# lr40/marl-scheduling

Measured on AMD Instinct MI355X. Metric: agent-env-steps/sec (whole node), 8 agents×8 cores×16384 envs, 1/2/4/8 MI355X, higher is better.
Workload: dtype int8/f32

## Files before the change

marl-scheduling_amd/csrc/env_kernels.hip:

```cpp
#include <hip/hip_runtime.h>
#include <stdlib.h>
#include <string.h>

#include "ms_layout.h"
#include "ms_act.h"

#pragma clang fp contract(off)

namespace ms {

__device__ __forceinline__ void wave_sync() {
    __builtin_amdgcn_fence(__ATOMIC_RELEASE, "wavefront");
    __builtin_amdgcn_wave_barrier();
    __builtin_amdgcn_fence(__ATOMIC_ACQUIRE, "wavefront");
}

#ifdef MS_PHASE_TIMING
constexpr int kProbeSlots = 65536;
__device__ unsigned long long g_phase_cycles[kProbeSlots][16];
__device__ unsigned long long g_wave_span[kProbeSlots][2];
__device__ unsigned long long g_free_cycles[kProbeSlots][5];
#define MS_MARK(k)                                                     \
    do {                                                               \
        const uint64_t t_now = __builtin_amdgcn_s_memtime();          \
        t_acc[k] += t_now - t_prev;                                    \
        t_prev = t_now;                                                \
    } while (0)
#else
#define MS_MARK(k) \
    do {           \
    } while (0)
#endif

template <int LPE>
struct Lanes {
    int gl;
    int gbase;
    __device__ explicit Lanes(int lane) : gl(lane & (LPE - 1)), gbase(lane & ~(LPE - 1)) {}
    __device__ __forceinline__ uint64_t ballot(bool p) const {
        const uint64_t m = __ballot(p);
        return LPE == 64 ? m : (m >> gbase) & ((1ull << (LPE & 63)) - 1ull);
    }
    __device__ __forceinline__ uint32_t shfl(uint32_t v, int src) const { return (uint32_t)__shfl((int)v, gbase + src); }
};


__device__ __forceinline__ uint32_t mt_temper(uint32_t y) {
    y ^= (y >> 11);
    y ^= (y << 7) & 0x9d2c5680u;
    y ^= (y << 15) & 0xefc60000u;
    y ^= (y >> 18);
    return y;
}

__device__ __forceinline__ uint32_t mt_step(uint32_t hi_src, uint32_t lo_src, uint32_t xsrc) {
    const uint32_t y = (hi_src & 0x80000000u) | (lo_src & 0x7fffffffu);
    return xsrc ^ (y >> 1) ^ ((y & 1u) ? 0x9908b0dfu : 0u);
}

__device__ __forceinline__ void mt_phase_range(int ph, int& lo, int& hi) {
    lo = ph * (kMtN - kMtM);
    hi = ph < 2 ? (ph + 1) * (kMtN - kMtM) : kMtN - 1;
}

__device__ void mt_twist_lds_wave(uint32_t* st, int lane) {
    for (int ph = 0; ph < 3; ph++) {
        int lo, hi;
        mt_phase_range(ph, lo, hi);
        for (int c0 = lo; c0 < hi; c0 += kWave) {
            const int i = c0 + lane;
            uint32_t v = 0;
            if (i < hi) v = mt_step(st[i], st[i + 1], st[ph == 0 ? i + kMtM : i + (kMtM - kMtN)]);
            wave_sync();
            if (i < hi) st[i] = v;
            wave_sync();
        }
    }
    if (lane == 0) st[kMtN - 1] = mt_step(st[kMtN - 1], st[0], st[kMtM - 1]);
    wave_sync();
}

__device__ void mt_twist_into_successor(uint32_t* mt_env, uint32_t sel, uint8_t* lds, int lane) {
    uint32_t* st = reinterpret_cast<uint32_t*>(lds);
    const uint32_t h = sel & 1u;
    const uint32_t* cur = mt_env + h * kMtN;
    uint32_t* nxt = mt_env + (h ^ 1u) * kMtN;
    for (int i = lane; i < kMtN; i += kWave) st[i] = cur[i];
    wave_sync();
    mt_twist_lds_wave(st, lane);
    for (int i = lane; i < kMtN; i += kWave) nxt[i] = st[i];
    __builtin_amdgcn_fence(__ATOMIC_RELEASE, "workgroup");
    __builtin_amdgcn_fence(__ATOMIC_ACQUIRE, "workgroup");
    wave_sync();
}

template <int LPE>
__device__ void mt_refill_groups(uint32_t* mt, int64_t e0, uint64_t need, uint32_t sel, uint8_t* lds, int lane) {
    while (need) {
        const int src = __ffsll((unsigned long long)need) - 1;
        need &= need - 1;
        mt_twist_into_successor(mt + (e0 + src / LPE) * 2 * kMtN, (uint32_t)__shfl((int)sel, src), lds, lane);
    }
}

template <int LPE>
__device__ void mt_refill_next(uint32_t* mt, const uint8_t* recs, const Geom& P, int64_t slot, bool active,
                               uint8_t* lds, int lane) {
    const int gl = lane & (LPE - 1);
    const int64_t e0 = slot * (kWave / LPE);
    uint32_t sel = 0;
    if (active && gl == 0) sel = *reinterpret_cast<const uint32_t*>(recs + (e0 + lane / LPE) * P.rec_bytes + 12);
    mt_refill_groups<LPE>(mt, e0, __ballot(active && gl == 0 && !(sel & 2u)), sel, lds, lane);
}

__device__ __forceinline__ void mt_commit(int fin, int32_t* mti, uint32_t* sel) {
    const uint32_t h = *sel & 1u;
    if (fin > 2 * kMtN) {
        *sel = h;
        *mti = fin - 2 * kMtN;
    } else if (fin > kMtN) {
        *sel = h ^ 1u;
        *mti = fin - kMtN;
    } else {
        *sel = h | 2u;
        *mti = fin;
    }
}

__device__ __forceinline__ uint32_t mt_ld(const uint32_t* p) {
    return __hip_atomic_load(const_cast<uint32_t*>(p), __ATOMIC_RELAXED, __HIP_MEMORY_SCOPE_AGENT);
}
__device__ __forceinline__ void mt_st(uint32_t* p, uint32_t v) {
    __hip_atomic_store(p, v, __ATOMIC_RELAXED, __HIP_MEMORY_SCOPE_AGENT);
}

template <int LPE>
__device__ void mt_twist_from(uint32_t* cur, const uint32_t* nxt, int gl) {
    for (int i = gl; i < kMtN; i += LPE) mt_st(cur + i, nxt[i]);
    __builtin_amdgcn_fence(__ATOMIC_ACQ_REL, "workgroup");
    for (int ph = 0; ph < 3; ph++) {
        int lo, hi;
        mt_phase_range(ph, lo, hi);
        for (int c0 = lo; c0 < hi; c0 += LPE) {
            const int i = c0 + gl;
            uint32_t v = 0;
            if (i < hi) v = mt_step(mt_ld(cur + i), mt_ld(cur + i + 1), mt_ld(cur + (ph == 0 ? i + kMtM : i + (kMtM - kMtN))));
            __builtin_amdgcn_fence(__ATOMIC_ACQ_REL, "workgroup");
            if (i < hi) mt_st(cur + i, v);
            __builtin_amdgcn_fence(__ATOMIC_ACQ_REL, "workgroup");
        }
    }
    if (gl == 0) mt_st(cur + kMtN - 1, mt_step(mt_ld(cur + kMtN - 1), mt_ld(cur), mt_ld(cur + kMtM - 1)));
    __builtin_amdgcn_fence(__ATOMIC_ACQ_REL, "workgroup");
}

template <int LPE>
struct MtStream {
    uint32_t* cur;
    uint32_t* nxt;
    int mti0;
    int wb, wend;
    int p;
    bool fell_back;
    bool overrun;
    bool store;
    uint32_t v;

    __device__ void init(uint32_t* mt_env, uint32_t sel, int mti, bool active) {
        cur = mt_env + (sel & 1u) * kMtN;
        nxt = mt_env + ((sel & 1u) ^ 1u) * kMtN;
        mti0 = mti;
        wb = wend = p = 0;
        fell_back = false;
        overrun = false;
        store = active;
// ... 1368 lines not shown
        const int owner = (int)reinterpret_cast<const int8_t*>(sl + g.s_rec + g.o_core_owner)[c];
        const bool v = ge < EPW && e < E && owner > 0;
        const uint32_t* crow = reinterpret_cast<const uint32_t*>(sl + g.s_scratch) + c * nw;
        const int c0 = 2 * g4, c1 = 2 * g4 + 1;
        const u4v x = bytes_to_bf16(crow[c0 < nw ? c0 : nw - 1], crow[c1 < nw ? c1 : nw - 1]);
        acc_a[0] = (f4){0, 0, 0, 0};
        acc_a[0] = mfma_bf16(wa.hi[0], x, acc_a[0]);
        acc_a[0] = mfma_bf16(wa.mid[0], x, acc_a[0]);
        acc_a[0] = mfma_bf16(wa.lo[0], x, acc_a[0]);
        acc_a[1] = acc_a[0];
        const int64_t item = e * Ua + (owner - 1) * C + c;
        u_a[0] = philox_u(item, fa.acc.row_base, fa.acc_offset);
        u_a[1] = 0.f;
        row_a[0] = v ? (int)item : -1;
        row_a[1] = -1;
    }
    ho.run2(acc_o, Ao, g4, u_o, act_o, lp_o);
    ha.run2(acc_a, Aa, g4, u_a, act_a, lp_a);
    store(fa.off_action, fa.off_logprob, row_o, act_o, lp_o);
    store(fa.acc_action, fa.acc_logprob, row_a, act_a, lp_a);
    for (int t0 = 32; t0 < EPW * Uo; t0 += 32) {
        offer_rows(t0, acc_o, row_o, u_o);
        ho.run2(acc_o, Ao, g4, u_o, act_o, lp_o);
        store(fa.off_action, fa.off_logprob, row_o, act_o, lp_o);
    }
    const float S = __uint_as_float(s_tab[0]);
    const int last_nz = (int)s_tab[1];
    {
        const int ge = lane / Ua, u = lane - ge * Ua, a = u / C, c = u - a * C;
        const int64_t e = e0 + ge;
        const uint8_t* sl = smem_all + (size_t)(ge < EPW ? ge : 0) * g.s_total;
        const bool in = lane < EPW * Ua && e < E;
        const int owner = (int)reinterpret_cast<const int8_t*>(sl + g.s_rec + g.o_core_owner)[c];
        if (in && owner != a + 1) {
            const int64_t item = e * Ua + u;
            const float target = philox_u(item, fa.acc.row_base, fa.acc_offset) * S;
            int cnt = 0;
#pragma unroll
            for (int step = 16; step >= 1; step >>= 1)
                if (cnt + step <= 16 && s_cum[cnt + step - 1] <= target) cnt += step;
            const int act = cnt >= Aa ? last_nz : cnt;
            fa.acc_action[item] = (int8_t)act;
            fa.acc_logprob[item] = s_lp[act];
        }
    }
}

template <int LPE, bool EXT, bool CMP, class SH>
__global__ void __launch_bounds__(64, 4) k_env_step(Params P, int64_t E, uint8_t* recs, uint32_t* mt, Liab* liab,
                                                 StepIO io) {
#ifdef MS_PHASE_TIMING
    const uint64_t rt_start = __builtin_amdgcn_s_memrealtime();
#endif
    if (io.span && threadIdx.x == 0) {
        io.span[4 * blockIdx.x] = __builtin_amdgcn_s_memrealtime();
        io.span[4 * blockIdx.x + 2] = __builtin_amdgcn_s_memtime();
    }
    env_round<LPE, EXT, CMP, SH>(P, E, recs, mt, liab, io, blockIdx.x);
    if (io.span && threadIdx.x == 0) {
        io.span[4 * blockIdx.x + 3] = __builtin_amdgcn_s_memtime();
        io.span[4 * blockIdx.x + 1] = __builtin_amdgcn_s_memrealtime();
    }
#ifdef MS_PHASE_TIMING
    if (threadIdx.x == 0) {
        g_wave_span[blockIdx.x % kProbeSlots][0] = rt_start;
        g_wave_span[blockIdx.x % kProbeSlots][1] = __builtin_amdgcn_s_memrealtime();
    }
#endif
}

template <int LPE, class SH, bool MET = false>
__global__ void __launch_bounds__(64, 4) k_env_step_act(Params P, int64_t E, uint8_t* recs, uint32_t* mt, Liab* liab,
                                                     StepIO io, FusedAct fa) {
    if (io.span && threadIdx.x == 0) {
        io.span[4 * blockIdx.x] = __builtin_amdgcn_s_memrealtime();
        io.span[4 * blockIdx.x + 2] = __builtin_amdgcn_s_memtime();
    }
    env_round<LPE, false, true, SH, MET>(P, E, recs, mt, liab, io, blockIdx.x);
    fused_act<LPE, SH>(P, E, fa, blockIdx.x);
    if (io.span && threadIdx.x == 0) {
        io.span[4 * blockIdx.x + 3] = __builtin_amdgcn_s_memtime();
        io.span[4 * blockIdx.x + 1] = __builtin_amdgcn_s_memrealtime();
    }
}

template <class T>
__device__ __forceinline__ T* advance(T* p, int64_t bytes) {
    return p ? reinterpret_cast<T*>(reinterpret_cast<uintptr_t>(p) + bytes) : p;
}
struct RolloutArgs {
    Params P;
    int64_t E;
    uint8_t* recs;
    uint32_t* mt;
    Liab* liab;
    StepIO io;
    FusedAct fa;
    RoundStride st;
    int n_rounds, act_last;
};
template <int LPE, class SH, bool MET = false>
__global__ void __launch_bounds__(64, 2) k_env_rollout_act(RolloutArgs A0) {
    unsigned long long* span = A0.io.span;
    if (span && threadIdx.x == 0) {
        span[4 * blockIdx.x] = __builtin_amdgcn_s_memrealtime();
        span[4 * blockIdx.x + 2] = __builtin_amdgcn_s_memtime();
    }
    const int n_rounds = A0.n_rounds;
    for (int t = 0; t < n_rounds; t++) {
        auto ka = __builtin_amdgcn_kernarg_segment_ptr();
        asm volatile("" : "+s"(ka));
        const RolloutArgs& A = *(const RolloutArgs*)ka;
        int lane = threadIdx.x;
        asm volatile("" : "+v"(lane));
        const RoundStride& st = A.st;
        StepIO io = A.io;
        io.span = nullptr;
        io.act_acc = advance(io.act_acc, t * st.act_acc);
        io.act_off = advance(io.act_off, t * st.act_off);
        io.obs_crow = advance(io.obs_crow, t * st.obs_crow);
        io.obs_cown = advance(io.obs_cown, t * st.obs_cown);
        io.obs_off = advance(io.obs_off, t * st.obs_off);
        io.rew_offer = advance(io.rew_offer, t * st.rew_offer);
        io.rew_acc = advance(io.rew_acc, t * st.rew_acc);
        io.rew_agent = advance(io.rew_agent, t * st.rew_agent);
        io.rew_auct = advance(io.rew_auct, t * st.rew_auct);
        env_round<LPE, false, true, SH, MET, MET>(A.P, A.E, A.recs, A.mt, A.liab, io, blockIdx.x, lane);
        if (t + 1 < n_rounds || A.act_last) {
            FusedAct fa = A.fa;
            fa.off_action = advance(fa.off_action, t * st.off_action);
            fa.off_logprob = advance(fa.off_logprob, t * st.off_logprob);
            fa.acc_action = advance(fa.acc_action, t * st.acc_action);
            fa.acc_logprob = advance(fa.acc_logprob, t * st.acc_logprob);
            fa.off_offset += (uint64_t)t * st.offset_step;
            fa.acc_offset += (uint64_t)t * st.offset_step;
            fused_act<LPE, SH>(A.P, A.E, fa, blockIdx.x, lane);
        }
        __builtin_amdgcn_fence(__ATOMIC_RELEASE, "workgroup");
        __builtin_amdgcn_fence(__ATOMIC_ACQUIRE, "workgroup");
        wave_sync();
    }
    if (span && threadIdx.x == 0) {
        span[4 * blockIdx.x + 3] = __builtin_amdgcn_s_memtime();
        span[4 * blockIdx.x + 1] = __builtin_amdgcn_s_memrealtime();
    }
}

constexpr int kPriceTW1 = 36;

__device__ __forceinline__ uint32_t pick4u(const uint32_t (&v)[4], int k) {
    return k == 0 ? v[0] : (k == 1 ? v[1] : (k == 2 ? v[2] : v[3]));
}

template <class SH, int PART = 3>
__device__ __forceinline__ void act_free(const Geom& g, int64_t E, const FusedActFree& fa, int64_t e0, int a, int lane,
                                         uint8_t* lds, const FreeLds& fl, bool pace_on = false) {
    const int j = lane & 15, g4 = lane >> 4;
    const int partner = a ^ 4;
    const bool pacing = pace_on && partner < g.N;
    auto pace = [&]() {
        if (!pacing) return;
        volatile int* pg = reinterpret_cast<volatile int*>(lds + fl.pace);
        const int mine = pg[a] + 1;
        pg[a] = mine;
        const int other = __builtin_amdgcn_readfirstlane(pg[partner]);
        if (other > __builtin_amdgcn_readfirstlane(mine))
            __builtin_amdgcn_s_setprio(1);
        else
            __builtin_amdgcn_s_setprio(0);
    };
    const int N = g.N, C = g.C, L = g.L, Uo = g.NL, Ua = N * C;
    const int EW = kFreeEPW * N;
    const uint64_t dev_off = fa.offset_dev ? *fa.offset_dev : 0ull;
    const int16_t* pdig = reinterpret_cast<const int16_t*>(lds + fl.pdig);
    auto slice = [&](int k) -> const uint8_t* { return lds + k * g.s_total; };

    if constexpr ((PART & 1) != 0) {
        using FL = FragLayout<1, 1>;
        constexpr int TW = kPriceTW1;
        W1Split<1> w1;
        Head<1> h1;
        if (const uint32_t* fg = frag_groups<1, 1>(fa.core, false)) {
            const uint32_t* lf = fg + (size_t)a * FL::GB + lane * FL::LW;
            w1.load_frag(lf);
            h1.load_frag(reinterpret_cast<const float*>(lf + 12));
        } else {
            w1.load(fa.core.w1 + (size_t)a * 16 * fa.core.in_dim, fa.core.in_dim, j, g4);
            h1.load(fa.core, a, j, g4);
        }
        const int n_rows = EW * L, tiles = (n_rows + 15) >> 4;
        const uint64_t off = fa.off_offset + dev_off;
        const uint32_t rbase = (uint32_t)fa.core.row_base;
        const long long rows_all = E * Uo;
        const RawBuf ca_b(fa.core_action, rows_all), cl_b(fa.core_logprob, 4 * rows_all),
            ps_b(fa.price_state, 4 * rows_all), pa_b(fa.price_action, rows_all), pl_b(fa.price_logprob, 4 * rows_all),
            ep_b(fa.env_price, rows_all);
        const RawBuf tab_b(fa.ptab + (size_t)a * fa.pkeys * TW, 4ll * fa.pkeys * TW);
        const int nwo = g.off_stride >> 2, pcol = (2 * C) >> 2, pshift = 8 * ((2 * C) & 3);
        const int A1 = fa.core.n_actions, A2 = fa.price.n_actions;
        auto row_of = [&](int r, int& k, int& s) -> int {
            k = r / L;
            s = r - k * L;
            const bool v = r < n_rows && e0 + k < E;
            const int row = (int)((e0 + k) * Uo) + a * L + s;
            if (r >= n_rows) k = s = 0;
            return v ? row : -1;
        };
        uint32_t rb0[4] = {0, 0, 0, 0}, rb1[4] = {0, 0, 0, 0};
        auto core_pair = [&](int tile, int (&cur)[2], int (&act)[2], float (&lp)[2], float (&u2)[2], int (&pin)[2],
                             int (&dg)[2]) {
            if ((tile & 3) == 0) {
                int k, s;
                const int r = row_of(16 * (tile + g4) + j, k, s);
                uint32_t r0, r1;
                philox2((uint32_t)r + rbase, off, fa.seed, r0, r1);
                rows_bcast(r1, rb1);
                rows_bcast(r0, rb0);
            }
            const int kq = tile & 3;
            int kk[2], ss[2];
            f4 acc[2];
            float u1[2];
#pragma unroll
            for (int i = 0; i < 2; i++) {
                cur[i] = row_of(16 * (tile + i) + j, kk[i], ss[i]);
                const uint8_t* sc = slice(kk[i]) + g.s_scratch;
                const uint32_t* otmpl = reinterpret_cast<const uint32_t*>(sc + g.s_otmpl);
                const uint32_t pr = reinterpret_cast<const uint16_t*>(sc + g.s_slotpair)[a * L + ss[i]];
                uint32_t d[2];
#pragma unroll
                for (int h = 0; h < 2; h++) {
                    const int cc = 2 * g4 + h, wd = cc < nwo ? cc : nwo - 1;
                    d[h] = otmpl[wd] | (wd == pcol ? pr << pshift : 0u);
                }
                const u4v x = bytes_to_bf16(d[0], d[1]);
                acc[i] = (f4){0, 0, 0, 0};
                acc[i] = mfma_bf16(w1.hi[0], x, acc[i]);
                acc[i] = mfma_bf16(w1.mid[0], x, acc[i]);
                acc[i] = mfma_bf16(w1.lo[0], x, acc[i]);
                u1[i] = u24(pick4u(rb0, kq + i));
                u2[i] = u24(pick4u(rb1, kq + i));
            }
            h1.run2(acc, A1, g4, u1, act, lp);
#pragma unroll
            for (int i = 0; i < 2; i++) {
                const int kb = g4 < 2 ? 2 * act[i] + g4 : 2 * C + (g4 - 2);
                const int8_t* sc = reinterpret_cast<const int8_t*>(slice(kk[i]) + g.s_scratch);
                const int byte = kb < 2 * C ? sc[g.s_otmpl + kb] : sc[g.s_slotpair + 2 * (a * L + ss[i]) + (kb - 2 * C)];
                pin[i] = act[i] == 0 ? -5 : byte;
                dg[i] = cur[i] >= 0 ? (int)pdig[g4 * 256 + pin[i] + 128] : 0;
            }
        };
        auto price_out = [&](const int (&cur)[2], const int (&act)[2], const int (&pin)[2], const int (&pact)[2],
                             const float (&plp)[2]) {
#pragma unroll
            for (int i = 0; i < 2; i++)
                if (cur[i] >= 0) {
                    const uint32_t pc = (uint32_t)cur[i];
                    ps_b.st8(4 * pc + g4, pin[i]);
                    if (g4 == 0) {
                        pa_b.st8(pc, pact[i]);
                        pl_b.stf(4 * pc, plp[i]);
                        ep_b.st8(pc, act[i] == 0 ? -5 : pact[i]);
                    }
                }
        };
        bool any_miss = false;
        for (int tile = 0; tile < tiles; tile += 2) {
            int cur[2], act[2], pin[2], dg[2];
            float lp[2], u2[2];
            core_pair(tile, cur, act, lp, u2, pin, dg);
            if (__ballot(dg[0] < 0 || dg[1] < 0) == 0ull) {
                rows_sum2_i(dg[0], dg[1]);
                float cum[2][4], S2[2];
                int lnz[2], cnt[2], pact[2];
                float plp[2];
                uint32_t te[2];
#pragma unroll
                for (int i = 0; i < 2; i++) {
                    te[i] = __umul24((uint32_t)dg[i], 4u * TW);
                    const auto c4 = __builtin_amdgcn_raw_buffer_load_b128(tab_b.r, (int)(te[i] + 4 * (4 * g4)), 0, 0);
#pragma unroll
                    for (int q = 0; q < 4; q++) cum[i][q] = __uint_as_float(c4[q]);
                    S2[i] = tab_b.ldf(te[i] + 4 * 32);
                    lnz[i] = (int)tab_b.ld32(te[i] + 4 * 33);
                }
#pragma unroll
                for (int i = 0; i < 2; i++) {
                    const float target = u2[i] * S2[i];
                    cnt[i] = 0;
#pragma unroll
                    for (int q = 0; q < 4; q++) cnt[i] += (cum[i][q] <= target) ? 1 : 0;
                }
                rows_sum2_i(cnt[0], cnt[1]);
#pragma unroll
                for (int i = 0; i < 2; i++) {
                    pact[i] = cnt[i] >= A2 ? lnz[i] : cnt[i];
                    plp[i] = tab_b.ldf(te[i] + 4 * (16 + pact[i]));
                }
                price_out(cur, act, pin, pact, plp);
            } else {
                any_miss = true;
            }
#pragma unroll
            for (int i = 0; i < 2; i++)
                if (cur[i] >= 0 && g4 == 0) {
                    ca_b.st8((uint32_t)cur[i], act[i]);
                    cl_b.stf(4 * (uint32_t)cur[i], lp[i]);
                }
            pace();
        }
        if (any_miss) {
            Head<1> h2;
            h2.load(fa.price, a, j, g4);
            const float pw1 = fa.price.w1[((size_t)a * 16 + j) * 4 + g4];
            for (int tile = 0; tile < tiles; tile += 2) {
                int cur[2], act[2], pin[2], dg[2];
                float lp[2], u2[2];
                core_pair(tile, cur, act, lp, u2, pin, dg);
// ... 202 lines not shown
constexpr int kFillRounds = 8;
template <bool PAIR>
__global__ void __launch_bounds__(256) k_acc_common_fill4(CommonFillArgs p, int n_acts, int merge) {
    __shared__ __align__(16) float tabs[8 * kFreeTabDw];
    using FL = FragLayout<2, 2>;
    for (int k = threadIdx.x; k < p.N * kFreeTabDw; k += blockDim.x) {
        const int a = k / kFreeTabDw;
        tabs[k] = __uint_as_float(p.frag[(size_t)a * FL::GB + 64 * FL::LW + (k - a * kFreeTabDw)]);
    }
    __syncthreads();
    const int C = p.C, U = p.N * C, QR = U >> 2;
    const uint32_t g = (uint32_t)blockIdx.x * 256 + threadIdx.x;
    const uint32_t pr = __umulhi(g, magic_div((uint32_t)QR)), uq = g - pr * (uint32_t)QR;
    const uint32_t S = PAIR ? 64u / (uint32_t)C : 1u;
    const uint32_t e0 = PAIR ? (((pr & ~(S - 1u)) << 1) | (pr & (S - 1u))) : pr, e1 = e0 + S;
    if (e0 >= (uint32_t)p.E) return;
    const bool has1 = PAIR && e1 < (uint32_t)p.E;
    const int u = 4 * (int)uq, a = small_div(u, C), c0 = u - a * C;
    uint32_t row[4], hi = 0;
#pragma unroll
    for (int k = 0; k < 4; k++) {
        if constexpr (PAIR) {
            row[k] = e0 * (uint32_t)U + (uint32_t)(u + k) + p.row_base;
        } else {
            const uint32_t i = e0 * (uint32_t)C + (uint32_t)(c0 + k), ib = i & ~64u;
            const uint32_t eb = C == 1 ? ib : __umulhi(ib, magic_div((uint32_t)C));
            row[k] = eb * (uint32_t)U + (uint32_t)(a * C) + (ib - eb * (uint32_t)C) + p.row_base;
            hi |= ((i >> 6) & 1u) << k;
        }
    }
    const float* tab = tabs + a * kFreeTabDw;
    const float tmax = tab[64];
    float bm[3];
#pragma unroll
    for (int b = 0; b < 3; b++) bm[b] = tab[8 * b + 7];
    const int t0 = (int)blockIdx.y * kFillRounds;
    uint32_t own0[kFillRounds], own1[kFillRounds];
#pragma unroll
    for (int j = 0; j < kFillRounds; j++) {
        const int8_t* ob = advance(p.owner, (int64_t)(t0 + j) * p.owner_stride);
        own0[j] = t0 + j < n_acts ? *reinterpret_cast<const uint32_t*>(ob + (size_t)e0 * C + c0) : 0u;
        own1[j] = has1 && t0 + j < n_acts ? *reinterpret_cast<const uint32_t*>(ob + (size_t)e1 * C + c0) : 0u;
    }
    const uint64_t off0 = p.offset + (p.offset_dev ? *p.offset_dev : 0ull);
    const uint32_t mine = 0x01010101u * (uint32_t)(a + 1);
    auto store = [&](uint32_t e, int t, int owned, uint32_t acts, const float (&lps)[4]) {
        const size_t r = (size_t)e * U + u;
        int8_t* ad = advance(p.action, (int64_t)t * p.action_stride) + r;
        float* ld = advance(p.logprob, (int64_t)t * p.logprob_stride) + r;
        if (owned == 0 || merge || p.own_action) {
            uint32_t a4 = acts;
            float4 l4 = make_float4(lps[0], lps[1], lps[2], lps[3]);
            if (owned != 0) {
                const size_t oc = (size_t)e * C + c0;
                const uint32_t old_a = p.own_action
                                           ? *reinterpret_cast<const uint32_t*>(advance(p.own_action, (int64_t)t * p.own_action_stride) + oc)
                                           : *reinterpret_cast<const uint32_t*>(ad);
                const float4 old_l = p.own_action
                                         ? *reinterpret_cast<const float4*>(advance(p.own_logprob, (int64_t)t * p.own_logprob_stride) + oc)
                                         : *reinterpret_cast<const float4*>(ld);
                uint32_t m = 0;
#pragma unroll
                for (int k = 0; k < 4; k++) m |= ((owned >> k) & 1) ? 0xffu << (8 * k) : 0u;
                a4 = (acts & ~m) | (old_a & m);
                if (owned & 1) l4.x = old_l.x;
                if (owned & 2) l4.y = old_l.y;
                if (owned & 4) l4.z = old_l.z;
                if (owned & 8) l4.w = old_l.w;
            }
            *reinterpret_cast<uint32_t*>(ad) = a4;
            *reinterpret_cast<float4*>(ld) = l4;
        } else {
#pragma unroll
            for (int k = 0; k < 4; k++)
                if (!((owned >> k) & 1)) {
                    ad[k] = (int8_t)(acts >> (8 * k));
                    ld[k] = lps[k];
                }
        }
    };
#pragma unroll
    for (int j = 0; j < kFillRounds; j++) {
        const int t = t0 + j;
        if (t >= n_acts) break;
        const uint64_t off = off0 + (uint64_t)t * p.offset_step;
        const uint32_t x0 = own0[j] ^ mine, x1 = has1 ? own1[j] ^ mine : 0u;
        int owned0 = 0, owned1 = 0;
#pragma unroll
        for (int k = 0; k < 4; k++) {
            owned0 |= ((x0 >> (8 * k)) & 0xffu) == 0u ? 1 << k : 0;
            owned1 |= ((x1 >> (8 * k)) & 0xffu) == 0u ? 1 << k : 0;
        }
        constexpr int NI = PAIR ? 8 : 4;
        float tg[NI];
        int cnt[NI];
#pragma unroll
        for (int k = 0; k < 4; k++) {
            uint32_t w0, w1;
            philox2(row[k], off, p.seed, w0, w1);
            tg[k] = u24(PAIR ? w0 : (((hi >> k) & 1u) ? w1 : w0)) * tmax;
            if constexpr (PAIR) tg[4 + k] = u24(w1) * tmax;
        }
#pragma unroll
        for (int i = 0; i < NI; i++) {
            int nb = 0;
#pragma unroll
            for (int b = 0; b < 3; b++) nb += bm[b] <= tg[i] ? 1 : 0;
            cnt[i] = nb;
        }
        float4 blo[NI], bhi[NI];
#pragma unroll
        for (int i = 0; i < NI; i++) {
            blo[i] = *reinterpret_cast<const float4*>(tab + 8 * cnt[i]);
            bhi[i] = *reinterpret_cast<const float4*>(tab + 8 * cnt[i] + 4);
        }
#pragma unroll
        for (int i = 0; i < NI; i++) {
            const float t = tg[i];
            cnt[i] = 8 * cnt[i] + (blo[i].x <= t) + (blo[i].y <= t) + (blo[i].z <= t) + (blo[i].w <= t) + (bhi[i].x <= t) +
                     (bhi[i].y <= t) + (bhi[i].z <= t) + (bhi[i].w <= t);
        }
        const int lnz = __float_as_int(tab[65]);
        uint32_t acts0 = 0, acts1 = 0;
        float lps0[4], lps1[4];
#pragma unroll
        for (int k = 0; k < 4; k++) {
            const int a0 = cnt[k] >= p.A ? lnz : cnt[k];
            acts0 |= (uint32_t)(uint8_t)a0 << (8 * k);
            lps0[k] = tab[32 + a0];
            if constexpr (PAIR) {
                const int a1 = cnt[4 + k] >= p.A ? lnz : cnt[4 + k];
                acts1 |= (uint32_t)(uint8_t)a1 << (8 * k);
                lps1[k] = tab[32 + a1];
            } else {
                lps1[k] = 0.f;
            }
        }
        store(e0, t, owned0, acts0, lps0);
        if (has1) store(e1, t, owned1, acts1, lps1);
    }
}

struct RolloutFreeArgs {
    Params P;
    int64_t E;
    uint8_t* recs;
    uint32_t* mt;
    Liab* liab;
    StepIO io;
    FusedActFree fa;
    RoundStrideFree st;
    int n_rounds, act_last;
    int prio;
};
template <class SH, bool MET = false>
__global__ void __launch_bounds__(512, 4) k_env_rollout_act_free(RolloutFreeArgs A0) {
    extern __shared__ __align__(16) uint8_t smem_free[];
    Geom g;
    if constexpr (SH::kStatic) {
        constexpr Geom kg = make_geom(SH::kN, SH::kC, SH::kL, SH::kJ);
        g = kg;
    } else {
        g = A0.P;
    }
    const int wave = __builtin_amdgcn_readfirstlane((int)(threadIdx.x >> 6));
    const int lane0 = (int)threadIdx.x & 63;
    const FreeLds fl = free_lds(g);
    const int64_t wslot = (int64_t)blockIdx.x * g.N + wave;
    unsigned long long* span = A0.io.span;
    if (span && lane0 == 0) {
        span[4 * wslot] = __builtin_amdgcn_s_memrealtime();
        span[4 * wslot + 2] = __builtin_amdgcn_s_memtime();
    }
    {
        uint32_t* pd = reinterpret_cast<uint32_t*>(smem_free + fl.pdig);
        const uint32_t* src = reinterpret_cast<const uint32_t*>(A0.fa.pdigit);
        for (int k = (int)threadIdx.x; k < 512; k += (int)blockDim.x) pd[k] = src[k];
        uint32_t* ax = reinterpret_cast<uint32_t*>(smem_free + fl.accx);
        for (int k = (int)threadIdx.x; k < (fl.total - fl.accx) / 4; k += (int)blockDim.x) ax[k] = 0u;
    }
    __syncthreads();
#ifdef MS_PHASE_TIMING
    uint64_t f_prev = __builtin_amdgcn_s_memtime(), f_acc[5] = {0, 0, 0, 0, 0};
#define FREE_MARK(k)                                                   \
    do {                                                               \
        const uint64_t f_now = __builtin_amdgcn_s_memtime();          \
        if ((k) >= 0) f_acc[(k) < 0 ? 0 : (k)] += f_now - f_prev;      \
        f_prev = f_now;                                                \
    } while (0)
#else
#define FREE_MARK(k) \
    do {             \
    } while (0)
#endif
    const int n_rounds = A0.n_rounds;
    for (int t = 0; t < n_rounds; t++) {
        auto ka = __builtin_amdgcn_kernarg_segment_ptr();
        asm volatile("" : "+s"(ka));
        const RolloutFreeArgs& A = *(const RolloutFreeArgs*)ka;
        int lane = (int)threadIdx.x & 63;
        asm volatile("" : "+v"(lane));
        const RoundStrideFree& st = A.st;
        StepIO io = A.io;
        io.span = nullptr;
        io.act_acc = advance(io.act_acc, t * st.act_acc);
        io.act_off = advance(io.act_off, t * st.act_off);
        io.obs_crow = advance(io.obs_crow, t * st.obs_crow);
        io.obs_cown = advance(io.obs_cown, t * st.obs_cown);
        io.obs_off = advance(io.obs_off, t * st.obs_off);
        io.rew_offer = advance(io.rew_offer, t * st.rew_offer);
        io.rew_price = advance(io.rew_price, t * st.rew_price);
        io.rew_acc = advance(io.rew_acc, t * st.rew_acc);
        io.rew_agent = advance(io.rew_agent, t * st.rew_agent);
        io.rew_auct = advance(io.rew_auct, t * st.rew_auct);
        FREE_MARK(-1);
        const bool up = wave >= 4 && (A.prio & 2);
        if (up) __builtin_amdgcn_s_setprio(1);
        const int8_t* acc_lds = t > 0 && A.fa.own_action
                                    ? reinterpret_cast<const int8_t*>(smem_free + fl.accx) + wave * kFreeEPW * g.N * g.C
                                    : nullptr;
        env_round<kWave / kFreeEPW, false, true, SH, MET, MET>(A.P, A.E, A.recs, A.mt, A.liab, io, wslot, lane,
                                                               smem_free + wave * free_slot(g), acc_lds);
        if (up) __builtin_amdgcn_s_setprio(0);
        FREE_MARK(0);
        if (t + 1 < n_rounds || A.act_last) {
            __syncthreads();
            FREE_MARK(1);
            FusedActFree fa = A.fa;
            fa.core_action = advance(fa.core_action, t * st.core_action);
            fa.core_logprob = advance(fa.core_logprob, t * st.core_logprob);
            fa.price_state = advance(fa.price_state, t * st.price_state);
            fa.price_action = advance(fa.price_action, t * st.price_action);
            fa.price_logprob = advance(fa.price_logprob, t * st.price_logprob);
            fa.acc_action = advance(fa.acc_action, t * st.acc_action);
            fa.acc_logprob = advance(fa.acc_logprob, t * st.acc_logprob);
            fa.own_action = advance(fa.own_action, t * st.own_action);
            fa.own_logprob = advance(fa.own_logprob, t * st.own_logprob);
            fa.off_offset += (uint64_t)t * st.offset_step;
            fa.acc_offset += (uint64_t)t * st.offset_step;
            const bool up_act = wave >= 4 && (A.prio & 1);
            if (up_act) __builtin_amdgcn_s_setprio(1);
            const bool pace_on = (A.prio & 4) != 0;
#ifdef MS_PHASE_TIMING
            act_free<SH, 1>(g, A.E, fa, (int64_t)blockIdx.x * kFreeEPW * g.N, wave, lane, smem_free, fl, pace_on);
            FREE_MARK(2);
            act_free<SH, 2>(g, A.E, fa, (int64_t)blockIdx.x * kFreeEPW * g.N, wave, lane, smem_free, fl, pace_on);
#else
            act_free<SH>(g, A.E, fa, (int64_t)blockIdx.x * kFreeEPW * g.N, wave, lane, smem_free, fl, pace_on);
#endif
            if (up_act || pace_on) __builtin_amdgcn_s_setprio(0);
            FREE_MARK(3);
            __syncthreads();
            FREE_MARK(4);
        }
    }
    if (span && lane0 == 0) {
        span[4 * wslot + 3] = __builtin_amdgcn_s_memtime();
        span[4 * wslot + 1] = __builtin_amdgcn_s_memrealtime();
    }
#ifdef MS_PHASE_TIMING
    if (lane0 == 0)
        for (int k = 0; k < 5; k++) g_free_cycles[wslot % kProbeSlots][k] += f_acc[k];
#endif
}

__global__ void __launch_bounds__(64) k_env_auctioneer(Params P, uint8_t* recs, uint32_t* mt, int8_t* actions) {
    extern __shared__ __align__(16) uint8_t smem[];
    M128* s_mc = reinterpret_cast<M128*>(smem + P.s_mc);
    M128* s_mr = reinterpret_cast<M128*>(smem + P.s_mr);
    int16_t* s_auct = reinterpret_cast<int16_t*>(smem + P.s_auct);
    const int lane = threadIdx.x;
    const Lanes<kWave> Lg(lane);
    const int64_t e = blockIdx.x;
    uint8_t* rec = smem + P.s_rec;
    __shared__ int32_t s_kt[48];
    mt_refill_next<kWave>(mt, recs, P, blockIdx.x, true, smem, lane);
    load_kind_tables(P, s_kt, lane);
    copy_dwords<kWave>(reinterpret_cast<uint32_t*>(rec),
                       reinterpret_cast<const uint32_t*>(recs + e * (int64_t)P.rec_bytes), P.rec_bytes / 4, lane);
    wave_sync();
    Rec R{rec, &P, s_kt};
    MtStream<kWave> rs;
    rs.init(mt + e * 2 * kMtN, R.mt_sel(), R.mti(), true);
    rs.load(0, 0, Lg);
    build_masks<kWave>(R, P, s_mc, s_mr, lane);
    hardcoded_auctioneer<kWave>(R, P, s_mc, s_mr, rs, s_auct, Lg);
    wave_sync();
    for (int c = lane; c < P.C; c += kWave) actions[e * P.C + c] = (int8_t)s_auct[c];
    if (lane == 0) {
        int32_t* hdr = reinterpret_cast<int32_t*>(recs + e * (int64_t)P.rec_bytes);
        mt_commit(rs.end_index(), hdr + 2, reinterpret_cast<uint32_t*>(hdr + 3));
    }
}

__global__ void __launch_bounds__(64) k_env_randbelow(Params P, uint8_t* recs, uint32_t* mt, int64_t e, uint32_t n,
                                                      uint32_t* out) {
    extern __shared__ __align__(16) uint8_t smem[];
    const int lane = threadIdx.x;
    const Lanes<kWave> Lg(lane);
    uint8_t* rec = recs + e * (int64_t)P.rec_bytes;
    int32_t* mti = reinterpret_cast<int32_t*>(rec + 8);
    uint32_t* sel = reinterpret_cast<uint32_t*>(rec + 12);
    if (!(*sel & 2u)) mt_twist_into_successor(mt + e * 2 * kMtN, *sel, smem, lane);
    MtStream<kWave> rs;
    rs.init(mt + e * 2 * kMtN, *sel, *mti, true);
    const uint32_t r = rs.randbelow(n, Lg);
    wave_sync();
    if (lane == 0) {
        *out = r;
        mt_commit(rs.end_index(), mti, sel);
    }
}

}

#ifdef MS_PHASE_TIMING
extern "C" int ms_probe_phase_cycles(unsigned long long* out, int clear) {
    static unsigned long long host[ms::kProbeSlots][16];
    if (hipMemcpyFromSymbol(host, HIP_SYMBOL(ms::g_phase_cycles), sizeof(host)) != hipSuccess) return -1;
    for (int k = 0; k < 16; k++) {
        out[k] = 0;
        for (int b = 0; b < ms::kProbeSlots; b++) out[k] += host[b][k];
    }
    if (clear) {
        memset(host, 0, sizeof(host));
        if (hipMemcpyToSymbol(HIP_SYMBOL(ms::g_phase_cycles), host, sizeof(host)) != hipSuccess) return -1;
    }
    return 0;
}
extern "C" int ms_probe_phase_blocks(unsigned long long* out, int n_blocks) {
    static unsigned long long host[ms::kProbeSlots][16];
    if (n_blocks > ms::kProbeSlots) return -1;
    if (hipMemcpyFromSymbol(host, HIP_SYMBOL(ms::g_phase_cycles), sizeof(host)) != hipSuccess) return -1;
    memcpy(out, host, sizeof(unsigned long long) * 16 * n_blocks);
    return 0;
}
extern "C" int ms_probe_free_cycles(unsigned long long* out, int n_waves, int clear) {
    static unsigned long long host[ms::kProbeSlots][5];
    if (n_waves > ms::kProbeSlots) return -1;
    if (hipMemcpyFromSymbol(host, HIP_SYMBOL(ms::g_free_cycles), sizeof(host)) != hipSuccess) return -1;
    memcpy(out, host, sizeof(unsigned long long) * 5 * n_waves);
    if (clear) {
        memset(host, 0, sizeof(host));
        if (hipMemcpyToSymbol(HIP_SYMBOL(ms::g_free_cycles), host, sizeof(host)) != hipSuccess) return -1;
    }
    return 0;
}
extern "C" int ms_probe_wave_spans(unsigned long long* out, int n_blocks) {
    static unsigned long long host[ms::kProbeSlots][2];
    if (n_blocks > ms::kProbeSlots) return -1;
    if (hipMemcpyFromSymbol(host, HIP_SYMBOL(ms::g_wave_span), sizeof(host)) != hipSuccess) return -1;
    memcpy(out, host, sizeof(unsigned long long) * 2 * n_blocks);
    return 0;
}
#endif

namespace ms {
hipError_t launch_env_init(const Params& P, int64_t E, uint8_t* recs, uint32_t* mt, Liab* liab, uint64_t seed,
                           hipStream_t s) {
    const size_t lds = (size_t)P.s_scratch + 4 * kMtN > (size_t)P.s_total ? (size_t)P.s_scratch + 4 * kMtN : P.s_total;
    hipLaunchKernelGGL(k_env_init, dim3((unsigned)E), dim3(kWave), lds, s, P, recs, mt, liab, seed);
    return hipGetLastError();
}
hipError_t launch_env_reset(const Params& P, int64_t E, const uint8_t* recs, int8_t* a, int8_t* o, int8_t* u,
                            int8_t* crow, int8_t* cown, hipStream_t s) {
    hipLaunchKernelGGL(k_env_reset, dim3((unsigned)E), dim3(kWave), P.s_total, s, P, recs, a, o, u, crow, cown);
    return hipGetLastError();
}

#ifndef MS_MIN_LPE
#define MS_MIN_LPE 16
#endif
static int lanes_per_env(const Params& P, int64_t E) {
    int need = P.C > P.N ? P.C : P.N;
    int lpe = MS_MIN_LPE;
    while (lpe < need) lpe *= 2;
    static const long long min_waves = [] {
        const char* v = getenv("MS_ENV_MIN_WAVES");
        return v ? atoll(v) : 2048LL;
    }();
    while (E >= 1024 && lpe < kWave && (E * lpe + kWave - 1) / kWave < min_waves &&
           (E * 2 * lpe + kWave - 1) / kWave <= min_waves)
        lpe *= 2;
    return lpe;
}

template <int LPE, class SH>
static hipError_t launch_step_sh(const Params& P, int64_t E, uint8_t* recs, uint32_t* mt, Liab* liab, const StepIO& io,
                                 hipStream_t s) {
    constexpr int G = kWave / LPE;
    const int64_t blocks = (E + G - 1) / G;
    const size_t lds = (size_t)P.s_total * G > 4 * kMtN ? (size_t)P.s_total * G : 4 * kMtN;
    const bool compact = io.obs_crow != nullptr || io.obs_cown != nullptr;
    const bool ext = io.act_acc == nullptr || io.metrics != nullptr || (compact && io.obs_acc != nullptr);
    auto kern = ext ? k_env_step<LPE, true, false, DynShape>
                    : (compact ? k_env_step<LPE, false, true, SH> : k_env_step<LPE, false, false, SH>);
    hipLaunchKernelGGL(kern, dim3((unsigned)blocks), dim3(kWave), lds, s, P, E, recs, mt, liab, io);
    return hipGetLastError();
}

template <int N, int C, int L, int J>
static bool is_shape(const Params& P) {
    return P.N == N && P.C == C && P.L == L && P.new_jobs == J;
}

template <int LPE>
static hipError_t launch_step_t(const Params& P, int64_t E, uint8_t* recs, uint32_t* mt, Liab* liab, const StepIO& io,
                                hipStream_t s) {
#ifndef MS_NO_FIXED_SHAPES
    if constexpr (LPE == 16) {
        if (is_shape<8, 8, 3, 1>(P)) return launch_step_sh<LPE, FixShape<8, 8, 3, 1>>(P, E, recs, mt, liab, io, s);
        if (is_shape<16, 16, 3, 1>(P)) return launch_step_sh<LPE, FixShape<16, 16, 3, 1>>(P, E, recs, mt, liab, io, s);
    }
    if constexpr (LPE == 32) {
        if (is_shape<4, 4, 3, 1>(P)) return launch_step_sh<LPE, FixShape<4, 4, 3, 1>>(P, E, recs, mt, liab, io, s);
        if (is_shape<32, 32, 3, 1>(P)) return launch_step_sh<LPE, FixShape<32, 32, 3, 1>>(P, E, recs, mt, liab, io, s);
    }
#endif
    return launch_step_sh<LPE, DynShape>(P, E, recs, mt, liab, io, s);
}

hipError_t launch_env_step(const Params& P, int64_t E, uint8_t* recs, uint32_t* mt, Liab* liab, const StepIO& io,
                           hipStream_t s) {
    switch (lanes_per_env(P, E)) {
#if MS_MIN_LPE <= 8
        case 8: return launch_step_t<8>(P, E, recs, mt, liab, io, s);
#endif
        case 16: return launch_step_t<16>(P, E, recs, mt, liab, io, s);
        case 32: return launch_step_t<32>(P, E, recs, mt, liab, io, s);
        default: return launch_step_t<64>(P, E, recs, mt, liab, io, s);
    }
}
bool env_step_act_supported(const Params& P, int64_t E) {
    const int epw = kWave / lanes_per_env(P, E);
    return epw * P.N * P.C <= kWave && epw * P.NL <= kWave && epw * P.C <= 16;
}
template <int LPE, class SH>
static hipError_t launch_step_act_sh(const Params& P, int64_t E, uint8_t* recs, uint32_t* mt, Liab* liab,
                                     const StepIO& io, const FusedAct& fa, hipStream_t s) {
    constexpr int G = kWave / LPE;
    const int64_t blocks = (E + G - 1) / G;
    const size_t lds = (size_t)P.s_total * G > 4 * kMtN ? (size_t)P.s_total * G : 4 * kMtN;
    auto kern = io.metrics ? k_env_step_act<LPE, SH, true> : k_env_step_act<LPE, SH, false>;
    hipLaunchKernelGGL(kern, dim3((unsigned)blocks), dim3(kWave), lds, s, P, E, recs, mt, liab, io, fa);
    return hipGetLastError();
}
hipError_t launch_env_step_act(const Params& P, int64_t E, uint8_t* recs, uint32_t* mt, Liab* liab, const StepIO& io,
                               const FusedAct& fa, hipStream_t s) {
    if (!env_step_act_supported(P, E) || io.act_acc == nullptr || io.obs_acc != nullptr) return hipErrorInvalidValue;
    switch (lanes_per_env(P, E)) {
        case 16: return launch_step_act_sh<16, DynShape>(P, E, recs, mt, liab, io, fa, s);
        case 32:
#ifndef MS_NO_FIXED_SHAPES
            if (is_shape<4, 4, 3, 1>(P)) return launch_step_act_sh<32, FixShape<4, 4, 3, 1>>(P, E, recs, mt, liab, io, fa, s);
#endif
            return launch_step_act_sh<32, DynShape>(P, E, recs, mt, liab, io, fa, s);
        default: return launch_step_act_sh<64, DynShape>(P, E, recs, mt, liab, io, fa, s);
    }
}
template <int LPE, class SH>
static hipError_t launch_rollout_act_sh(const Params& P, int64_t E, uint8_t* recs, uint32_t* mt, Liab* liab,
                                        const StepIO& io, const FusedAct& fa, const RoundStride& st, int n_rounds,
                                        int act_last, hipStream_t s) {
    constexpr int G = kWave / LPE;
    const int64_t blocks = (E + G - 1) / G;
    const size_t lds = (size_t)P.s_total * G > 4 * kMtN ? (size_t)P.s_total * G : 4 * kMtN;
    const RolloutArgs A{P, E, recs, mt, liab, io, fa, st, n_rounds, act_last};
    auto kern = io.metrics ? k_env_rollout_act<LPE, SH, true> : k_env_rollout_act<LPE, SH, false>;
    hipLaunchKernelGGL(kern, dim3((unsigned)blocks), dim3(kWave), lds, s, A);
    return hipGetLastError();
}
hipError_t launch_env_rollout_act(const Params& P, int64_t E, uint8_t* recs, uint32_t* mt, Liab* liab,
                                  const StepIO& io, const FusedAct& fa, const RoundStride& st, int n_rounds,
                                  int act_last, hipStream_t s) {
    if (!env_step_act_supported(P, E) || io.act_acc == nullptr || io.obs_acc != nullptr || io.ev_acc != nullptr ||
        io.ev_term != nullptr || n_rounds < 1)
        return hipErrorInvalidValue;
    switch (lanes_per_env(P, E)) {
        case 16: return launch_rollout_act_sh<16, DynShape>(P, E, recs, mt, liab, io, fa, st, n_rounds, act_last, s);
        case 32:
#ifndef MS_NO_FIXED_SHAPES
            if (is_shape<4, 4, 3, 1>(P))
                return launch_rollout_act_sh<32, FixShape<4, 4, 3, 1>>(P, E, recs, mt, liab, io, fa, st, n_rounds,
                                                                       act_last, s);
#endif
            return launch_rollout_act_sh<32, DynShape>(P, E, recs, mt, liab, io, fa, st, n_rounds, act_last, s);
        default: return launch_rollout_act_sh<64, DynShape>(P, E, recs, mt, liab, io, fa, st, n_rounds, act_last, s);
    }
}
bool env_rollout_free_supported(const Params& P) {
    return P.free_prices && free_rollout_shape_ok(P) && free_rollout_lds_ok(P);
}
template <class SH>
static hipError_t launch_rollout_free_sh(const Params& P, int64_t E, uint8_t* recs, uint32_t* mt, Liab* liab,
                                         const StepIO& io, const FusedActFree& fa, const RoundStrideFree& st,
                                         int n_rounds, int act_last, hipStream_t s) {
    const int64_t epb = (int64_t)kFreeEPW * P.N;
    const int64_t blocks = (E + epb - 1) / epb;
    static const int prio = [] {
        const char* v = getenv("MS_FREE_PRIO");
        return v ? atoi(v) : 4;
    }();
    const RolloutFreeArgs A{P, E, recs, mt, liab, io, fa, st, n_rounds, act_last, prio};
    auto kern = io.metrics ? k_env_rollout_act_free<SH, true> : k_env_rollout_act_free<SH, false>;
    hipLaunchKernelGGL(kern, dim3((unsigned)blocks), dim3(64 * P.N), (size_t)free_lds(P).total, s, A);
    return hipGetLastError();
}
static int fill_merge() {
    static const int v = [] {
        const char* e = getenv("MS_FILL_MERGE");
        return e && e[0] == '0' ? 0 : 1;
    }();
    return v;
}
static bool fill_pair_enabled() {
    static const bool v = [] {
        const char* e = getenv("MS_FILL_PAIR");
        return !(e && e[0] == '0');
    }();
    return v;
}
static bool fill_quad_enabled() {
    static const bool v = [] {
        const char* e = getenv("MS_FILL_QUAD");
        return !(e && e[0] == '0');
    }();
    return v;
}
void acc_common_tables(const void* act_frag, const uint32_t** tab0, int* group_dwords) {
    using FL = FragLayout<2, 2>;
    static_assert(FL::TB == kFreeTabDw, "common table size");
    *tab0 = static_cast<const uint32_t*>(act_frag) + 4 + 64 * FL::LW;
    *group_dwords = FL::GB;
}
hipError_t launch_env_fill_common(const Params& P, int64_t E, const StepIO& io, const FusedActFree& fa,
                                  const RoundStrideFree& st, int n_rounds, int act_last, hipStream_t s) {
    const int n_acts = act_last ? n_rounds : n_rounds - 1;
    if (!env_rollout_free_supported(P) || io.obs_cown == nullptr || fa.acc.act_frag == nullptr) return hipErrorInvalidValue;
    if (n_acts < 1) return hipSuccess;
    const CommonFillArgs c{io.obs_cown, fa.acc_action, fa.acc_logprob, st.obs_cown, st.acc_action, st.acc_logprob,
                           fa.own_action, fa.own_logprob, st.own_action, st.own_logprob,
                           static_cast<const uint32_t*>(fa.acc.act_frag) + 4, (int)E, P.N, P.C, fa.acc.n_actions,
                           (uint32_t)fa.acc.row_base, fa.seed, fa.acc_offset, st.offset_step, fa.offset_dev};
    const int64_t items = E * P.N * P.C;
    const bool quad = P.C % 4 == 0 && fill_quad_enabled() &&
                      ((reinterpret_cast<uintptr_t>(c.owner) | (uintptr_t)c.owner_stride) & 3) == 0 &&
                      ((reinterpret_cast<uintptr_t>(c.action) | (uintptr_t)c.action_stride) & 3) == 0 &&
                      ((reinterpret_cast<uintptr_t>(c.logprob) | (uintptr_t)c.logprob_stride) & 15) == 0 &&
                      ((reinterpret_cast<uintptr_t>(c.own_action) | (uintptr_t)c.own_action_stride) & 3) == 0 &&
                      ((reinterpret_cast<uintptr_t>(c.own_logprob) | (uintptr_t)c.own_logprob_stride) & 15) == 0;
    if (quad) {
        const unsigned by = (unsigned)((n_acts + kFillRounds - 1) / kFillRounds);
        const int64_t qr = (int64_t)P.N * P.C / 4;
        if (64 % P.C == 0 && fill_pair_enabled()) {
            const int64_t S = 64 / P.C, pairs = (E + 2 * S - 1) / (2 * S) * S;
            hipLaunchKernelGGL(k_acc_common_fill4<true>, dim3((unsigned)((pairs * qr + 255) / 256), by), dim3(256), 0, s,
                               c, n_acts, fill_merge());
        } else {
            hipLaunchKernelGGL(k_acc_common_fill4<false>, dim3((unsigned)((E * qr + 255) / 256), by), dim3(256), 0, s, c,
                               n_acts, fill_merge());
        }
        return hipGetLastError();
    }
    const unsigned bx = (unsigned)((items + kFillPer * 256 - 1) / (kFillPer * 256));
    hipLaunchKernelGGL(k_acc_common_fill, dim3(bx, (unsigned)n_acts), dim3(256), 0, s, c);
    return hipGetLastError();
}
hipError_t launch_env_rollout_act_free(const Params& P, int64_t E, uint8_t* recs, uint32_t* mt, Liab* liab,
                                       const StepIO& io, const FusedActFree& fa, const RoundStrideFree& st,
                                       int n_rounds, int act_last, hipStream_t s) {
    if (!env_rollout_free_supported(P) || io.act_acc == nullptr || io.obs_acc != nullptr || io.ev_acc != nullptr ||
        io.ev_term != nullptr || n_rounds < 1)
        return hipErrorInvalidValue;
#ifndef MS_NO_FIXED_SHAPES
    if (is_shape<8, 8, 3, 1>(P))
        return launch_rollout_free_sh<FixShape<8, 8, 3, 1>>(P, E, recs, mt, liab, io, fa, st, n_rounds, act_last, s);
#endif
    return launch_rollout_free_sh<DynShape>(P, E, recs, mt, liab, io, fa, st, n_rounds, act_last, s);
}
hipError_t launch_env_auctioneer(const Params& P, int64_t E, uint8_t* recs, uint32_t* mt, int8_t* actions,
                                 hipStream_t s) {
    const size_t lds = (size_t)P.s_total > 4 * kMtN ? (size_t)P.s_total : 4 * kMtN;
    hipLaunchKernelGGL(k_env_auctioneer, dim3((unsigned)E), dim3(kWave), lds, s, P, recs, mt, actions);
    return hipGetLastError();
}
hipError_t launch_env_randbelow(const Params& P, uint8_t* recs, uint32_t* mt, int64_t e, uint32_t n, uint32_t* out,
                                hipStream_t s) {
    hipLaunchKernelGGL(k_env_randbelow, dim3(1), dim3(kWave), 4 * kMtN, s, P, recs, mt, e, n, out);
    return hipGetLastError();
}
}
```

Before: 1.494 billion.

## Stagger co-resident free-rollout workgroups with per-CU tickets and time-sliced wave priorities

Adds a STAG variant of the free-price rollout kernel. Each workgroup takes a per-CU ticket through a global atomic to get a rank; with the default stagger mode (4) the waves get s_setprio 3 during the env step, and afterwards an alternating upper or lower priority chosen from a realtime-clock time slice XOR the pair id. Pacing inside act_free maps to priorities 2/3 for the upper group. The goal is to desynchronize workgroups that share a CU so their env and act phases overlap instead of contending. It also adds optional probe buffers for per-round timestamps and a ticket-sum readout, and it costs a global atomic, extra barriers and setprio churn on every round.

```diff
diff --git a/marl-scheduling_amd/csrc/env_kernels.hip b/marl-scheduling_amd/csrc/env_kernels.hip
--- a/marl-scheduling_amd/csrc/env_kernels.hip
+++ b/marl-scheduling_amd/csrc/env_kernels.hip
@@ -20,7 +20,9 @@
 __device__ unsigned long long g_phase_cycles[kProbeSlots][16];
 __device__ unsigned long long g_wave_span[kProbeSlots][2];
 __device__ unsigned long long g_free_cycles[kProbeSlots][5];
-#define MS_MARK(k)                                                     \
+constexpr int kProbeWgs = 4096, kProbeRoundsHead = 64, kProbeRoundsTail = 16;
+__device__ unsigned long long g_free_rounds[kProbeWgs][1 + kProbeRoundsHead + kProbeRoundsTail];
+#define MS_MARK(k)                                                    \
     do {                                                               \
         const uint64_t t_now = __builtin_amdgcn_s_memtime();          \
         t_acc[k] += t_now - t_prev;                                    \
@@ -1695,9 +1697,15 @@
     return k == 0 ? v[0] : (k == 1 ? v[1] : (k == 2 ? v[2] : v[3]));
 }
 
-template <class SH, int PART = 3>
+__device__ __forceinline__ bool stagger_upper_pair(int pair) {
+    if (pair < 2) return pair != 0;
+    const uint32_t slice = (uint32_t)(__builtin_amdgcn_s_memrealtime() >> ((pair >> 2) & 31));
+    return __builtin_amdgcn_readfirstlane((int)((slice ^ (uint32_t)pair) & 1u)) == 0;
+}
+template <class SH, int PART = 3, bool SEP = false>
 __device__ __forceinline__ void act_free(const Geom& g, int64_t E, const FusedActFree& fa, int64_t e0, int a, int lane,
-                                         uint8_t* lds, const FreeLds& fl, bool pace_on = false) {
+                                         uint8_t* lds, const FreeLds& fl, bool pace_on = false,
+                                         int prio_upper = 0) {
     const int j = lane & 15, g4 = lane >> 4;
     const int partner = a ^ 4;
     const bool pacing = pace_on && partner < g.N;
@@ -1707,7 +1715,19 @@
         const int mine = pg[a] + 1;
         pg[a] = mine;
         const int other = __builtin_amdgcn_readfirstlane(pg[partner]);
-        if (other > __builtin_amdgcn_readfirstlane(mine))
+        const bool behind = other > __builtin_amdgcn_readfirstlane(mine);
+        if constexpr (SEP) {
+            int upper = __builtin_amdgcn_readfirstlane(prio_upper);
+            asm volatile("" : "+s"(upper));
+            if (upper) {
+                if (behind)
+                    __builtin_amdgcn_s_setprio(3);
+                else
+                    __builtin_amdgcn_s_setprio(2);
+                return;
+            }
+        }
+        if (behind)
             __builtin_amdgcn_s_setprio(1);
         else
             __builtin_amdgcn_s_setprio(0);
@@ -2216,8 +2236,18 @@
     RoundStrideFree st;
     int n_rounds, act_last;
     int prio;
+    int stagger;
+    int stagger_delay;
+    int stagger_slice;
 };
-template <class SH, bool MET = false>
+constexpr int kCuKeys = 1 << 12;
+__device__ __forceinline__ uint32_t cu_key() {
+    const uint32_t cu = __builtin_amdgcn_s_getreg(4 | (8 << 6) | (7 << 11));
+    const uint32_t xcc = __builtin_amdgcn_s_getreg(20 | (3 << 11));
+    return (xcc << 8 | cu) & (kCuKeys - 1);
+}
+__device__ uint32_t g_cu_ticket[kCuKeys];
+template <class SH, bool MET = false, bool STAG = false>
 __global__ void __launch_bounds__(512, 4) k_env_rollout_act_free(RolloutFreeArgs A0) {
     extern __shared__ __align__(16) uint8_t smem_free[];
     Geom g;
@@ -2244,7 +2274,25 @@
         for (int k = (int)threadIdx.x; k < (fl.total - fl.accx) / 4; k += (int)blockDim.x) ax[k] = 0u;
     }
     __syncthreads();
+    [[maybe_unused]] int prio_pair = -1;
+    [[maybe_unused]] int rank = 0;
+    if constexpr (STAG) {
+        volatile int* pg = reinterpret_cast<volatile int*>(smem_free + fl.pace);
+        if (threadIdx.x == 0) pg[0] = (int)(atomicAdd(&g_cu_ticket[cu_key()], 1u) & 1u);
+        __syncthreads();
+        rank = __builtin_amdgcn_readfirstlane(pg[0]);
+        __syncthreads();
+        if (threadIdx.x == 0) pg[0] = 0;
+        if (rank != 0 && (A0.stagger & 1)) {
+            const uint64_t t0 = __builtin_amdgcn_s_memtime(), d = (uint64_t)(uint32_t)A0.stagger_delay;
+            while (__builtin_amdgcn_s_memtime() - t0 < d) __builtin_amdgcn_s_sleep(8);
+        }
+        if (A0.stagger & 6)
+            prio_pair = (A0.stagger & 4) ? (A0.stagger_slice & 31) << 2 | 2 | rank : (rank == 0 ? 1 : 0);
+    }
 #ifdef MS_PHASE_TIMING
+    if (threadIdx.x == 0 && blockIdx.x < kProbeWgs)
+        g_free_rounds[blockIdx.x][0] = 1ull << 63 | (unsigned long long)rank << 32 | cu_key();
     uint64_t f_prev = __builtin_amdgcn_s_memtime(), f_acc[5] = {0, 0, 0, 0, 0};
 #define FREE_MARK(k)                                                   \
     do {                                                               \
@@ -2280,16 +2328,38 @@
         FREE_MARK(-1);
         const bool up = wave >= 4 && (A.prio & 2);
         if (up) __builtin_amdgcn_s_setprio(1);
+        [[maybe_unused]] int prio_upper = 0;
+        if constexpr (STAG) {
+            prio_pair = __builtin_amdgcn_readfirstlane(prio_pair);
+            asm volatile("" : "+s"(prio_pair));
+            if (prio_pair >= 0) __builtin_amdgcn_s_setprio(3);
+        }
         const int8_t* acc_lds = t > 0 && A.fa.own_action
                                     ? reinterpret_cast<const int8_t*>(smem_free + fl.accx) + wave * kFreeEPW * g.N * g.C
                                     : nullptr;
         env_round<kWave / kFreeEPW, false, true, SH, MET, MET>(A.P, A.E, A.recs, A.mt, A.liab, io, wslot, lane,
                                                                smem_free + wave * free_slot(g), acc_lds);
         if (up) __builtin_amdgcn_s_setprio(0);
+        if constexpr (STAG) {
+            if (prio_pair >= 0) {
+                prio_upper = stagger_upper_pair(prio_pair) ? 1 : 0;
+                if (prio_upper)
+                    __builtin_amdgcn_s_setprio(2);
+                else
+                    __builtin_amdgcn_s_setprio(0);
+            }
+        }
         FREE_MARK(0);
         if (t + 1 < n_rounds || A.act_last) {
             __syncthreads();
             FREE_MARK(1);
+#ifdef MS_PHASE_TIMING
+            if (threadIdx.x == 0 && blockIdx.x < kProbeWgs) {
+                const int tail = t - (n_rounds - kProbeRoundsTail);
+                const int k = t < kProbeRoundsHead ? t : (tail >= 0 ? kProbeRoundsHead + tail : -1);
+                if (k >= 0) g_free_rounds[blockIdx.x][1 + k] = __builtin_amdgcn_s_memrealtime();
+            }
+#endif
             FusedActFree fa = A.fa;
             fa.core_action = advance(fa.core_action, t * st.core_action);
             fa.core_logprob = advance(fa.core_logprob, t * st.core_logprob);
@@ -2306,11 +2376,11 @@
             if (up_act) __builtin_amdgcn_s_setprio(1);
             const bool pace_on = (A.prio & 4) != 0;
 #ifdef MS_PHASE_TIMING
-            act_free<SH, 1>(g, A.E, fa, (int64_t)blockIdx.x * kFreeEPW * g.N, wave, lane, smem_free, fl, pace_on);
+            act_free<SH, 1, STAG>(g, A.E, fa, (int64_t)blockIdx.x * kFreeEPW * g.N, wave, lane, smem_free, fl, pace_on, prio_upper);
             FREE_MARK(2);
-            act_free<SH, 2>(g, A.E, fa, (int64_t)blockIdx.x * kFreeEPW * g.N, wave, lane, smem_free, fl, pace_on);
+            act_free<SH, 2, STAG>(g, A.E, fa, (int64_t)blockIdx.x * kFreeEPW * g.N, wave, lane, smem_free, fl, pace_on, prio_upper);
 #else
-            act_free<SH>(g, A.E, fa, (int64_t)blockIdx.x * kFreeEPW * g.N, wave, lane, smem_free, fl, pace_on);
+            act_free<SH, 3, STAG>(g, A.E, fa, (int64_t)blockIdx.x * kFreeEPW * g.N, wave, lane, smem_free, fl, pace_on, prio_upper);
 #endif
             if (up_act || pace_on) __builtin_amdgcn_s_setprio(0);
             FREE_MARK(3);
@@ -2378,6 +2448,14 @@
 
 }
 
+extern "C" long long ms_free_stagger_tickets(void) {
+    static uint32_t host[ms::kCuKeys];
+    if (hipMemcpyFromSymbol(host, HIP_SYMBOL(ms::g_cu_ticket), sizeof(host)) != hipSuccess) return -1;
+    long long n = 0;
+    for (int k = 0; k < ms::kCuKeys; k++) n += host[k];
+    return n;
+}
+
 #ifdef MS_PHASE_TIMING
 extern "C" int ms_probe_phase_cycles(unsigned long long* out, int clear) {
     static unsigned long long host[ms::kProbeSlots][16];
@@ -2415,6 +2493,14 @@
     if (n_blocks > ms::kProbeSlots) return -1;
     if (hipMemcpyFromSymbol(host, HIP_SYMBOL(ms::g_wave_span), sizeof(host)) != hipSuccess) return -1;
     memcpy(out, host, sizeof(unsigned long long) * 2 * n_blocks);
+    return 0;
+}
+extern "C" int ms_probe_free_rounds(unsigned long long* out, int n_wgs) {
+    constexpr int W = 1 + ms::kProbeRoundsHead + ms::kProbeRoundsTail;
+    static unsigned long long host[ms::kProbeWgs][W];
+    if (n_wgs > ms::kProbeWgs) return -1;
+    if (hipMemcpyFromSymbol(host, HIP_SYMBOL(ms::g_free_rounds), sizeof(host)) != hipSuccess) return -1;
+    memcpy(out, host, sizeof(unsigned long long) * W * n_wgs);
     return 0;
 }
 #endif
@@ -2555,6 +2641,8 @@
 bool env_rollout_free_supported(const Params& P) {
     return P.free_prices && free_rollout_shape_ok(P) && free_rollout_lds_ok(P);
 }
+constexpr int kFreeStaggerDefault = 4, kFreeStaggerSlice = 16;
+constexpr long kFreeStaggerDelay = 49000, kFreeStaggerDelayMax = 1 << 20;
 template <class SH>
 static hipError_t launch_rollout_free_sh(const Params& P, int64_t E, uint8_t* recs, uint32_t* mt, Liab* liab,
                                          const StepIO& io, const FusedActFree& fa, const RoundStrideFree& st,
@@ -2565,8 +2653,16 @@
         const char* v = getenv("MS_FREE_PRIO");
         return v ? atoi(v) : 4;
     }();
-    const RolloutFreeArgs A{P, E, recs, mt, liab, io, fa, st, n_rounds, act_last, prio};
-    auto kern = io.metrics ? k_env_rollout_act_free<SH, true> : k_env_rollout_act_free<SH, false>;
+    const char* sv = getenv("MS_FREE_STAGGER");
+    const int stagger = sv ? atoi(sv) & 7 : kFreeStaggerDefault;
+    const char* lv = getenv("MS_FREE_STAGGER_SLICE");
+    const int slice = lv ? atoi(lv) & 31 : kFreeStaggerSlice;
+    const char* dv = getenv("MS_FREE_STAGGER_DELAY");
+    long delay = dv ? atol(dv) : kFreeStaggerDelay;
+    delay = delay < 0 ? 0 : (delay > kFreeStaggerDelayMax ? kFreeStaggerDelayMax : delay);
+    const RolloutFreeArgs A{P, E, recs, mt, liab, io, fa, st, n_rounds, act_last, prio, stagger, (int)delay, slice};
+    auto kern = stagger ? (io.metrics ? k_env_rollout_act_free<SH, true, true> : k_env_rollout_act_free<SH, false, true>)
+                        : (io.metrics ? k_env_rollout_act_free<SH, true> : k_env_rollout_act_free<SH, false>);
     hipLaunchKernelGGL(kern, dim3((unsigned)blocks), dim3(64 * P.N), (size_t)free_lds(P).total, s, A);
     return hipGetLastError();
 }
```

Result: faster. 1.560 billion (median of 6 runs) (+4.4%).
